# Harrypotterrrr/DVD-GAN

Hardware: AMD Instinct MI355X
Metric: clips/sec per G+Ds+Dt step, 48x64x64 UCF-101 synth (higher is better)
Workload: dtype bf16; 1 GPU; UCF-101-shaped 101-class 48x64x64 clips, G+Ds+Dt hinge step, ch=32, k_sample=8, batch 64/GPU (BASELINE configs[1]); global_batch=64, parallelism=dp1

## Files before the change

### dvd_gan_amd/csrc/conv_wgrad.hip

```cpp
#include "conv_common.h"
#include "prof.h"
#include <cstdlib>
#include <type_traits>

namespace {

struct WgK {
    const char* x; const char* dy; float* dw;
    int M, C, ldx, Cin_real, Cout, Cy, ldy;
    int T, H, W, logH, logW, Hin, Win;
    int kt, kh, kw, up2, relu_in;
    int tiles_co, tiles_ci, rows_per_split;
    long long s_co, s_ci, s_tap;
    size_t x_bytes, dy_bytes;
    int maxshift, xcd_remap;
    float* dbias;
    float* wsb;
    float* ws;
    int fold, cout_f;
};

template <typename G>
__host__ __device__ __forceinline__ size_t ws_tile_off(size_t slice, G gx, int bx, int kw, int t, int tile_elems) { return ((slice * gx + bx) * kw + t) * (size_t)tile_elems; }
template <typename G>
// ... 3 lines not shown

__device__ __forceinline__ void xcd_block_remap(const WgK& p, int& bx, int& bz) {
    bx = blockIdx.x; bz = blockIdx.z;
    if (p.xcd_remap) {
        const int gx = gridDim.x, total = gx * gridDim.z, lin = bx + gx * bz;
        const int xcd = lin & 7, qd = total >> 3, rr = total & 7;
        const int lp = (xcd < rr ? xcd * (qd + 1) : rr * (qd + 1) + (xcd - rr) * qd) + (lin >> 3);
        bz = lp / gx; bx = lp - bz * gx;
    }
}
__device__ __forceinline__ void bf16x8_unpack(const u32x4& r, float (&v)[8]) {
    v[0] = __uint_as_float(r.x << 16); v[1] = __uint_as_float(r.x & 0xffff0000u);
    v[2] = __uint_as_float(r.y << 16); v[3] = __uint_as_float(r.y & 0xffff0000u);
    v[4] = __uint_as_float(r.z << 16); v[5] = __uint_as_float(r.z & 0xffff0000u);
    v[6] = __uint_as_float(r.w << 16); v[7] = __uint_as_float(r.w & 0xffff0000u);
}
#define WG_BIAS_FINISH(CPRA, RPPA, NV, TAB, TO_WS, N, I)                                                                \
    do {                                                                                                                \
        __syncthreads();                                                                                                \
        if (tid < CPRA) {                                                                                               \
            for (int k = 0; k < NV; ++k) {                                                                              \
                float a = 0.f;                                                                                          \
                for (int r = 0; r < RPPA; ++r) a += TAB;                                                                \
                const int co = co0 + tid * NV + k;                                                                      \
                if (TO_WS) p.wsb[ws_bias_off(bz, N, I, BMc) + tid * NV + k] = a;                                        \
                else if (co < p.Cout && a != 0.f) atomicAdd(p.dbias + co, a);      \
            }                                                                                                           \
        }                                                                                                               \
        __syncthreads();                                                                                                \
    } while (0)
#define WG_TILE_TAIL(ACC, ROW0, COL0, KW_, T, TAP)                                                                      \
    do {                                                                                                                \
        _Pragma("unroll") for (int r = 0; r < 16; ++r)                                                                  \
            ep[((r & 3) + 8 * (r >> 2) + 4 * (lane >> 5)) * 32 + (lane & 31)] = ACC[r];                                 \
        __builtin_amdgcn_s_waitcnt(0xc07f);                                                                             \
        __builtin_amdgcn_wave_barrier();                                                                                \
        const int ci = ci0 + COL0 + (lane & 31);                                                                        \
        const int cob = co0 + ROW0 + (lane >> 5);                                                                       \
        const int wtap = TAP;                   \
        if (p.ws) {                                                                                                     \
            float* wt = p.ws + ws_tile_off(bz, gridDim.x, bx, KW_, T, BMc * BNc) + (size_t)(ROW0) * BNc + COL0;         \
            _Pragma("unroll 1") for (int j = 0; j < 16; ++j)                                                            \
                wt[(size_t)(2 * j + (lane >> 5)) * BNc + (lane & 31)] = ep[(2 * j + (lane >> 5)) * 32 + (lane & 31)];   \
        } else if (ci < p.Cin_real) {                                                                                   \
            float* dst = p.dw + ci * p.s_ci + wtap * p.s_tap;                                                           \
            _Pragma("unroll 1") for (int j = 0; j < 16; ++j) {                                                          \
                const int co = cob + 2 * j;                                                                             \
                const float v = ep[(2 * j + (lane >> 5)) * 32 + (lane & 31)];                                           \
                if (co < p.Cout && v != 0.f) atomicAdd(dst + co * p.s_co, v);                                           \
            }                                                                                                           \
        }                                                                                                               \
        __builtin_amdgcn_wave_barrier();                                                                                \
    } while (0)
template <typename T, int TA, int TB>
__global__ __launch_bounds__(NT) void conv_wgrad_kernel(WgK p) {
    constexpr bool kBf16 = sizeof(T) == 2;
    static_assert(kBf16 || (TA == 2 && TB == 2), "exact mode uses the 128 x 128 tile");
    constexpr int BKW = kBf16 ? 32 : 16;
    constexpr int BMc = TA * 64, BNc = TB * 64;
    constexpr int RSA = BMc * 2 + 64, RSB = BNc * 2 + 64;
    constexpr int TA_BYTES = kBf16 ? 32 * RSA : TILEB, TB_BYTES = kBf16 ? 32 * RSB : TILEB;
    __shared__ __attribute__((aligned(16))) char smem[2][TA_BYTES + TB_BYTES];
    const int tid = threadIdx.x, lane = tid & 63, wave = tid >> 6;
    const int wm = wave >> 1, wn = wave & 1;
    int bx, bz;
    xcd_block_remap(p, bx, bz);
    const int tiles = p.tiles_co * p.tiles_ci;
    const int tap = bx / tiles;
    const int rem = bx - tap * tiles;
    const int tco = rem / p.tiles_ci, tci = rem - tco * p.tiles_ci;
    const int co0 = tco * BMc, ci0 = tci * BNc;
    const int it = tap / (p.kh * p.kw), r2 = tap - it * p.kh * p.kw;
    const int iy = r2 / p.kw, ix = r2 - iy * p.kw;
    const int dt = it - (p.kt >> 1), dy_ = iy - (p.kh >> 1), dx = ix - (p.kw >> 1);
    const int m_begin = bz * p.rows_per_split;
    const int m_end = min(p.M, m_begin + p.rows_per_split);

    f32x16 acc[TA][TB];
    {
        const f32x16 zacc = {0.f, 0.f, 0.f, 0.f, 0.f, 0.f, 0.f, 0.f, 0.f, 0.f, 0.f, 0.f, 0.f, 0.f, 0.f, 0.f};
#pragma unroll
        for (int a = 0; a < TA; ++a)
#pragma unroll
            for (int b = 0; b < TB; ++b) acc[a][b] = zacc;
    }

    constexpr unsigned ESZ = sizeof(T);
    const int xbase_row = p.up2 ? (m_begin / (p.H * p.W)) * p.Hin * p.Win : max(0, m_begin - p.maxshift);
    const size_t xbase_b = (size_t)xbase_row * p.ldx * ESZ, ybase_b = (size_t)m_begin * p.ldy * ESZ;
    const size_t xleft = p.x_bytes - xbase_b, yleft = p.dy_bytes > ybase_b ? p.dy_bytes - ybase_b : 0;
    const __amdgpu_buffer_rsrc_t rx = __builtin_amdgcn_make_buffer_rsrc(
        (void*)(p.x + xbase_b), 0, xleft > 0xfffffffeull ? 0xfffffffeu : (unsigned)xleft, 0x00020000);
    const __amdgpu_buffer_rsrc_t rdy = __builtin_amdgcn_make_buffer_rsrc(
        (void*)(p.dy + ybase_b), 0, yleft > 0xfffffffeull ? 0xfffffffeu : (unsigned)yleft, 0x00020000);
    const int delta = (dt * p.H + dy_) * p.W + dx;
    auto xoff = [&](int m, unsigned chan_bytes, bool cvalid) __attribute__((always_inline)) -> unsigned {
        int fm, ym, xm;
        grid_pos(m, p.H, p.W, p.logH, p.logW, fm, ym, xm);
        const int xx = xm + dx, yy = ym + dy_;
        int tt = dt;
        if (p.kt > 1) tt += fm % p.T;
        const bool ok = cvalid && m < m_end && (unsigned)yy < (unsigned)p.H && (unsigned)xx < (unsigned)p.W &&
                        (unsigned)tt < (unsigned)p.T;
        int row = m + delta;
        if (p.up2) row = ((fm + dt) * p.Hin + (yy >> 1)) * p.Win + (xx >> 1);
        return ok ? (unsigned)(row - xbase_row) * ((unsigned)p.ldx * ESZ) + chan_bytes : 0xffffffffu;
// ... 428 lines not shown
#pragma unroll
        for (int s_ = 0; s_ < NS; ++s_) mma1(&smem[buf * STAGE + s_ * SUB]);
    };
    if (m_begin < m_end) {
        const bool late = NWAVE == 8 && NS == 2 && wave >= 4;
        gload(m_begin);
        lstore(0);
        if (late) gload(m_begin + 32 * NS);
        __builtin_amdgcn_s_waitcnt(0xc07f);
        __builtin_amdgcn_s_barrier();
        int buf = 0;
        for (int mk = m_begin; mk < m_end; mk += 32 * NS, buf ^= 1) {
            if (!late) {
                gload(mk + 32 * NS);
                mma(buf);
                lstore(buf ^ 1);
            } else {
                mma1(&smem[buf * STAGE]);
                lstore(buf ^ 1);
                gload(mk + 2 * 32 * NS);
                mma1(&smem[buf * STAGE + (NS - 1) * SUB]);
            }
            __builtin_amdgcn_s_waitcnt(0xc07f);
            __builtin_amdgcn_s_barrier();
        }
        __builtin_amdgcn_s_waitcnt(0x0070);
    }
    if (do_bias) {
        float* red = reinterpret_cast<float*>(&smem[0]);
#pragma unroll
        for (int k = 0; k < 8; ++k) red[tid * 8 + k] = bs[k];
        WG_BIAS_FINISH(CPRA, RPPA, 8, red[(r * CPRA + tid) * 8 + k], spread, gridDim.x, bx);
    }
    float* ep = reinterpret_cast<float*>(&smem[0]) + wave * (32 * 32);
#pragma unroll
    for (int a = 0; a < 2; ++a)
#pragma unroll
        for (int t = 0; t < KW; ++t)
            WG_TILE_TAIL(acc[a][t], wm * 64 + a * 32, wn * 32, KW, t, irow * KW + t);
}
template <int I, int N, typename F>
__device__ __forceinline__ void static_for(F&& f) {
    if constexpr (I < N) {
        f(std::integral_constant<int, I>{});
        static_for<I + 1, N>(f);
    }
}
template <bool V>
__device__ __forceinline__ void mfma_pinned(f32x16& c, const bf16x8& a, const bf16x8& b) {
    if constexpr (V) asm volatile("v_mfma_f32_32x32x16_bf16 %0, %1, %2, %0" : "+v"(c) : "v"(a), "v"(b));
    else asm volatile("v_mfma_f32_32x32x16_bf16 %0, %1, %2, %0" : "+a"(c) : "v"(a), "v"(b));
}

#ifndef DVD_EXP_ROW4
#define DVD_EXP_ROW4 0
#endif
template <int KW, int AW, int BW, int WCO, int WCI, bool RELU, int DEPTH = 2, bool FOLD = false>
__global__ __launch_bounds__(256) void conv_wgrad_row4_kernel(WgK p) {
    constexpr bool BLDS = KW == 3 && AW * BW * KW > 16 && DEPTH >= 2;
    static_assert(WCO * WCI == 4, "four waves, one per SIMD");
    constexpr int NTt = 256, BMc = WCO * AW * 32, NHB = WCI * BW, BNc = NHB * 32;
    constexpr int RSA = BMc * 2 + 64;
    constexpr int TA_BYTES = 32 * RSA;
    constexpr int XROWS = KW == 5 ? 64 : 48, XHALF = XROWS * 64, TB_BYTES = NHB * XHALF;
    constexpr int SUB = TA_BYTES + TB_BYTES;
    constexpr int EPIB = 4 * 32 * 32 * 4, REDB = NTt * 8 * 4;
    constexpr int LDSB0 = 3 * SUB > EPIB ? (3 * SUB > REDB ? 3 * SUB : REDB) : (EPIB > REDB ? EPIB : REDB);
    constexpr int LDSB = LDSB0 + (BLDS ? REDB : 0);
    __shared__ __attribute__((aligned(16))) char smem[LDSB];
    const int tid = threadIdx.x, lane = tid & 63, wave = tid >> 6;
    const int wm = wave / WCI, wn = wave % WCI;
    int bx = blockIdx.x, bz = blockIdx.z;
    if (p.xcd_remap) {
        const int gx = gridDim.x, total = gx * gridDim.z, lin = bx + gx * bz;
        const int xcd = lin & 7, qd = total >> 3, rr = total & 7;
        const int lp = (xcd < rr ? xcd * (qd + 1) : rr * (qd + 1) + (xcd - rr) * qd) + (lin >> 3);
        bz = lp / gx; bx = lp - bz * gx;
    }
    const int tiles = p.tiles_co * p.tiles_ci;
    const int irow = bx / tiles;
    const int rem = bx - irow * tiles;
    const int tco = rem / p.tiles_ci, tci = rem - tco * p.tiles_ci;
    const int co0 = tco * BMc, ci0 = tci * BNc;
    constexpr int pad = KW >> 1;
    static_assert(!FOLD || (KW == 3 && BMc == 128), "the folded form runs on the 3-tap 128-channel tile");
    const int it = FOLD ? 0 : irow / KW, iy = FOLD ? irow : irow - it * KW;
    const int dyl = FOLD ? ((co0 / p.cout_f) >> 1) - 1 + irow : iy - pad, dtl = FOLD ? 0 : it - (p.kt >> 1);
    const int m_begin = bz * p.rows_per_split;
    const int m_end = min(p.M, m_begin + p.rows_per_split);

    f32x16 acc[AW][BW][KW];
    {
        const f32x16 zacc = {0.f, 0.f, 0.f, 0.f, 0.f, 0.f, 0.f, 0.f, 0.f, 0.f, 0.f, 0.f, 0.f, 0.f, 0.f, 0.f};
#pragma unroll
        for (int a = 0; a < AW; ++a)
#pragma unroll
            for (int b = 0; b < BW; ++b)
#pragma unroll
                for (int t = 0; t < KW; ++t) acc[a][b][t] = zacc;
    }
    const int xbase_row = max(0, m_begin - p.maxshift);
    const int ybase_row = FOLD ? 4 * m_begin - 2 * (p.W > 32 ? m_begin & (p.W - 1) : 0) : m_begin;
    const size_t xbase_b = (size_t)xbase_row * p.ldx * 2, ybase_b = (size_t)ybase_row * p.ldy * 2;
    const size_t xleft = p.x_bytes - xbase_b, yleft = p.dy_bytes > ybase_b ? p.dy_bytes - ybase_b : 0;
    const __amdgpu_buffer_rsrc_t rx = __builtin_amdgcn_make_buffer_rsrc(
        (void*)(p.x + xbase_b), 0, xleft > 0xfffffffeull ? 0xfffffffeu : (unsigned)xleft, 0x00020000);
    const __amdgpu_buffer_rsrc_t rdy = __builtin_amdgcn_make_buffer_rsrc(
        (void*)(p.dy + ybase_b), 0, yleft > 0xfffffffeull ? 0xfffffffeu : (unsigned)yleft, 0x00020000);
    const int segw = min(p.W, 32), logsegw = min(p.logW, 5);
    const int fpr = segw + KW - 1, frows = (32 >> logsegw) * fpr;
    constexpr int CPRA = BMc / 8, RPPA = NTt / CPRA, NPA = 32 / RPPA;
    const int rra = tid / CPRA, cka = tid % CPRA;
    const int cy = co0 + cka * 8;
    const bool cyv = cy < p.Cy;
    constexpr int CPX = NHB * 4;
    constexpr int NXL = (XROWS * CPX + NTt - 1) / NTt;
    constexpr int NOPS = NPA + NXL;
    constexpr bool XFULL = NXL * NTt == XROWS * CPX;
    int xa[NXL];
    static_assert(NTt % CPX == 0, "chunk i of a thread sits NTt / CPX footprint rows below chunk i - 1");
    const int xdst0 = ((tid % CPX) >> 2) * XHALF + (tid / CPX) * 64 + ((tid % CPX) & 3) * 16;
    unsigned xld[NXL];
    bool xv[NXL];
    const bool twofr = (32 >> logsegw) > p.H;
    const bool wide = p.W > 32;
    const unsigned ldx2 = (unsigned)p.ldx * 2, ldy2 = (unsigned)p.ldy * 2;
#pragma unroll
    for (int i = 0; i < NXL; ++i) {
        const int q = tid + i * NTt, row = q / CPX, c8 = q % CPX;
        const int seg = row / fpr, j = row - seg * fpr;
        const int cx = ci0 + c8 * 8;
        const int fo = twofr ? seg >> p.logH : 0, yl = twofr ? seg & (p.H - 1) : seg;
        const int xya = yl + dyl, xxa = j - pad;
        xa[i] = wide ? xxa : xya;
        xv[i] = row < frows && cx < p.C && (wide || (unsigned)xxa < (unsigned)p.W);
        const int delta = (fo << (p.logW + p.logH)) + (xya << p.logW) + xxa;
        xld[i] = (unsigned)delta * ldx2 + (unsigned)cx * 2;
    }
    unsigned yld = (unsigned)rra * ldy2 + (unsigned)cy * 2;
    unsigned ystep = (unsigned)RPPA * ldy2;
    if constexpr (FOLD) {
        static_assert(!FOLD || RPPA == 16, "16 rows per staging pass");
        const int ph = cy / p.cout_f, c = cy - ph * p.cout_f, W2 = 2 * p.W;
        yld = (unsigned)(((rra >> logsegw) * 2 + (ph >> 1)) * W2 + 2 * (rra & (segw - 1)) + (ph & 1)) * ldy2 + (unsigned)c * 2;
        ystep = (unsigned)(segw == 32 ? 32 : (16 >> logsegw) * 2 * W2) * ldy2;
    }
    const int dt_rows = p.kt > 1 ? dtl << (p.logW + p.logH) : 0;
    u32x4 R[DEPTH][NOPS];
    struct Geo { int sval; unsigned xoff, yoff; bool tok, ytok; };
    const unsigned slim = wide ? p.W : p.H;
    auto geo_part = [&](Geo& g, int mk, int part) __attribute__((always_inline)) {
        if (part == 0) {
            const int x0 = mk & (p.W - 1), y = twofr ? 0 : (mk >> p.logW) & (p.H - 1);
            g.sval = wide ? x0 : y;
            g.ytok = mk < m_end;
            g.tok = g.ytok && (!wide || (unsigned)(y + dyl) < (unsigned)p.H);
        } else if (part == 1) {
            if (p.kt > 1) {
                const int tt = (mk >> (p.logW + p.logH)) % p.T + dtl;
                g.tok = g.tok && (unsigned)tt < (unsigned)p.T;
            }
        } else if (part == 2) {
            g.xoff = (unsigned)(mk + dt_rows - xbase_row) * ldx2;
        } else {
// ... 43 lines not shown
            for (int k = 0; k < 8; ++k) {
                if constexpr (BLDS) __hip_atomic_fetch_add(btab + k * NTt, v8[k], __ATOMIC_RELAXED, __HIP_MEMORY_SCOPE_WORKGROUP);
                else bs[k] += v8[k];
            }
            return;
        }
        if (op < NPA) {
            *reinterpret_cast<u32x4*>(st + (rra + op * RPPA) * RSA + cka * 16) = R[op];
            if (mine) {
                float v[8];
                bf16x8_unpack(R[op], v);
#pragma unroll
                for (int k = 0; k < 8; ++k) {
                    if constexpr (BLDS) __hip_atomic_fetch_add(btab + k * NTt, v[k], __ATOMIC_RELAXED, __HIP_MEMORY_SCOPE_WORKGROUP);
                    else bs[k] += v[k];
                }
            }
        } else {
            const int i = op - NPA;
            if (XFULL || tid + i * NTt < XROWS * CPX)
                *reinterpret_cast<u32x4*>(st + TA_BYTES + xdst0 + i * (NTt / CPX) * 64) = RELU ? relu16_bf16(R[op]) : R[op];
        }
    };
    typedef __attribute__((ext_vector_type(4))) short s16x4;
    typedef __attribute__((ext_vector_type(8))) short s16x8;
    const int g16 = lane >> 4, i16 = lane & 15;
    const int frow = (g16 >> 1) * 8 + (i16 >> 2), fcol2 = ((g16 & 1) * 16 + (i16 & 3) * 4) * 2;
    auto tr2 = [&](const char* lo_, const char* hi_) __attribute__((always_inline)) -> bf16x8 {
        s16x4 lo = __builtin_amdgcn_ds_read_tr16_b64_v4i16((__attribute__((address_space(3))) s16x4*)lo_);
        s16x4 hi = __builtin_amdgcn_ds_read_tr16_b64_v4i16((__attribute__((address_space(3))) s16x4*)hi_);
        s16x8 f = __builtin_shufflevector(lo, hi, 0, 1, 2, 3, 4, 5, 6, 7);
        return __builtin_bit_cast(bf16x8, f);
    };
    const int fr0 = (frow >> logsegw) * fpr + (frow & (segw - 1));
    const int hlstep = (segw >= 8 ? 4 : fpr) * 64;
    const int kbstep = ((16 >> logsegw) * fpr + (16 & (segw - 1))) * 64;
    const int xoff0 = TA_BYTES + wn * BW * XHALF + fr0 * 64 + fcol2;
    const int aoff = frow * RSA + fcol2 + (wm * AW * 32) * 2;
    constexpr int UPK = KW * BW, NU = 2 * UPK;
    constexpr bool PIN = AW * BW * KW > 16;
    constexpr int UB = NU - 2;
    constexpr int RING = NU % 3 == 0 ? 3 : 5;
    static_assert(NU % RING == 0, "B fragment ring");
    bf16x8 fa[AW], fb[RING];
    auto ldA = [&](const char* st, int kb, int a) __attribute__((always_inline)) {
        const char* pz = st + aoff + kb * 16 * RSA + a * 64;
        fa[a] = tr2(pz, pz + 4 * RSA);
    };
    auto ldB = [&](const char* st, int u, int slot) __attribute__((always_inline)) {
        const int kb = u / UPK, t = (u % UPK) / BW, b = u % BW;
        const char* pz = st + xoff0 + kb * kbstep + t * 64 + b * XHALF;
        fb[slot] = tr2(pz, pz + hlstep);
    };
    if (m_begin < m_end) {
        {
            const Geo g0 = geo(m_begin);
#pragma unroll
            for (int op = 0; op < NOPS; ++op) load_op(op, g0, R[0]);
            const bool mine = do_bias && bphase == myshare;
            if (++bphase == nshare) bphase = 0;
#pragma unroll
            for (int op = 0; op < NOPS; ++op) store_op(op, &smem[0], mine, R[0]);
#pragma unroll
            for (int d = 0; d < DEPTH; ++d) {
                const Geo g1 = geo(m_begin + 32 * (d + 1));
#pragma unroll
                for (int op = 0; op < NOPS; ++op) load_op(op, g1, R[d]);
            }
            __builtin_amdgcn_s_waitcnt(0xc07f);
            __builtin_amdgcn_s_barrier();
#pragma unroll
            for (int a = 0; a < AW - 1; ++a) ldA(&smem[0], 0, a);
            ldB(&smem[0], 0, 0);
            ldB(&smem[0], 1, 1);
        }
        char* rd = &smem[0];
        char* nx = &smem[SUB];
        char* fr_ = &smem[2 * SUB];
        static_assert(AW == 4, "slot plan written for four A fragments per wave");
        Geo gl = geo(m_begin + 32 * (DEPTH + 1));
        for (int mk0 = m_begin; mk0 < m_end; mk0 += 32 * DEPTH) {
          static_for<0, DEPTH>([&](auto D_) __attribute__((always_inline)) {
            constexpr int dset = decltype(D_)::value;
            const int mk = mk0 + 32 * dset;
            const bool mine = do_bias && bphase == myshare;
            if (++bphase == nshare) bphase = 0;
            Geo gn = gl;
            __builtin_amdgcn_sched_barrier(0);
            static_for<0, NU * AW>([&](auto S_) __attribute__((always_inline)) {
                constexpr int s = decltype(S_)::value, u = s / AW, a = s % AW;
                constexpr int kb = u / UPK, t = (u % UPK) / BW, b = u % BW;
                if constexpr (u == UB && a == 0) {
                    __builtin_amdgcn_s_waitcnt(0xc07f);
                    if (!(DVD_EXP_ROW4 & 4)) __builtin_amdgcn_s_barrier();
                }
                if constexpr (a == 0) {
                    if (u + 2 < NU) ldB(rd, u + 2, (u + 2) % RING);
                    else ldB(nx, u + 2 - NU, (u + 2) % RING);
                }
                if constexpr (a == 1 || (ST64 && a == 2)) {
#pragma unroll
                    for (int op = 0; op < NOPS; ++op)
                        if ((op * UB) / NOPS == u && !(DVD_EXP_ROW4 & 2)) {
                            if constexpr (ST64) store_op(op, nx, mine, R[dset], a - 1);
                            else store_op(op, nx, mine, R[dset]);
                        }
                }
                if constexpr (u == UPK - 1 && a >= 1) ldA(rd, 1, a - 1);
                if constexpr (u == UPK && a == 0) ldA(rd, 1, AW - 1);
                if constexpr (u == NU - 1 && a >= 1) ldA(nx, 0, a - 1);
                if constexpr (u == 0 && a == 0) ldA(rd, 0, AW - 1);
                if constexpr (a == AW - 1) {
#pragma unroll
                    for (int op = 0; op < NOPS; ++op)
                        if ((op * UB) / NOPS == u && !(DVD_EXP_ROW4 & 1)) load_op(op, gl, R[dset]);
                }
                if constexpr (u == UB - 1 && a == AW - 1) geo_part(gn, mk + 32 * (DEPTH + 2), 0);
                if constexpr (u == UB && a >= 1) geo_part(gn, mk + 32 * (DEPTH + 2), a);
                if constexpr (PIN) mfma_pinned<((a * BW + b) * KW + t >= 16)>(acc[a][b][t], fa[a], fb[u % RING]);
                else acc[a][b][t] = __builtin_amdgcn_mfma_f32_32x32x16_bf16(fa[a], fb[u % RING], acc[a][b][t], 0, 0, 0);
                __builtin_amdgcn_sched_barrier(0);
            });
            gl = gn;
            char* t_ = rd; rd = nx; nx = fr_; fr_ = t_;
          });
        }
        __builtin_amdgcn_s_waitcnt(0x0070);
        if constexpr (PIN) asm volatile("s_nop 15\n\ts_nop 15" ::: "memory");
        __syncthreads();
    }
    if (do_bias) {
        if constexpr (!BLDS) {
#pragma unroll
            for (int k = 0; k < 8; ++k) btab[k * NTt] = bs[k];
        }
        WG_BIAS_FINISH(CPRA, RPPA, 8, btab[k * NTt + r * CPRA], spread, gridDim.x, bx);
    }
    float* ep = reinterpret_cast<float*>(&smem[0]) + wave * (32 * 32);
#pragma unroll
    for (int a = 0; a < AW; ++a)
#pragma unroll
        for (int b = 0; b < BW; ++b)
#pragma unroll
            for (int t = 0; t < KW; ++t)
                WG_TILE_TAIL(acc[a][b][t], (wm * AW + a) * 32, (wn * BW + b) * 32, KW, t, irow * KW + t);
}
#undef WG_BIAS_FINISH
#undef WG_TILE_TAIL
__device__ __forceinline__ f32x4 slice_sum4(const float* ws, int nslice, size_t stride, size_t off) {
    f32x4 a = {0.f, 0.f, 0.f, 0.f};
    int z = 0;
    for (; z + 4 <= nslice; z += 4) {
        f32x4 v[4];
#pragma unroll
        for (int j = 0; j < 4; ++j) v[j] = *reinterpret_cast<const f32x4*>(ws + (size_t)(z + j) * stride + off);
#pragma unroll
        for (int j = 0; j < 4; ++j) a += v[j];
    }
    for (; z < nslice; ++z) a += *reinterpret_cast<const f32x4*>(ws + (size_t)z * stride + off);
    return a;
}
__device__ __forceinline__ void wg_store4(float* d, long long s_ci, int ci, int Cin_real, const f32x4& a, int overwrite) {
#pragma unroll
    for (int j = 0; j < 4; ++j)
        if (ci + j < Cin_real) d[j * s_ci] = overwrite ? a[j] : d[j * s_ci] + a[j];
}
template <typename F>
__device__ __forceinline__ float block_sum_32x32(int nitem, F&& item) {
    __shared__ float red[32][33];
    const int c = threadIdx.x & 31, l = threadIdx.x >> 5;
    float a = 0.f;
    for (int i = l; i < nitem; i += 32 * 8) {
        float v[8];
#pragma unroll
        for (int u = 0; u < 8; ++u) v[u] = i + 32 * u < nitem ? item(i + 32 * u) : 0.f;
#pragma unroll
        for (int u = 0; u < 8; ++u) a += v[u];
    }
    red[l][c] = a;
    __syncthreads();
    if (l == 0)
        for (int j = 1; j < 32; ++j) a += red[j][c];
    return a;
}

struct WgRowRedK { const float* ws; float* dw; int nslice, gx, tiles_co, tiles_ci, BMc, BNc, KW, Cout, Cin_real; long long s_co, s_ci, s_tap; int overwrite; };
__global__ void wgrad_row_reduce_kernel(WgRowRedK p) {
    const int tile = p.BMc * p.BNc, tile_elems = p.KW * tile;
    const long long i = ((long long)blockIdx.x * blockDim.x + threadIdx.x) * 4;
    if (i >= (long long)p.gx * tile_elems) return;
    const int bx = (int)(i / tile_elems), e = (int)(i - (long long)bx * tile_elems);
    const int t = e / tile, e2 = e - t * tile;
    const int r = e2 / p.BNc, c = e2 - r * p.BNc;
    const int tiles = p.tiles_co * p.tiles_ci;
    const int iy = bx / tiles, rem = bx - iy * tiles;
    const int tco = rem / p.tiles_ci, tci = rem - tco * p.tiles_ci;
    const int co = tco * p.BMc + r, ci = tci * p.BNc + c;
    if (co >= p.Cout || ci >= p.Cin_real) return;
    const f32x4 a = slice_sum4(p.ws, p.nslice, ws_slice_stride(p.gx, p.KW, tile), ws_tile_off(0, p.gx, bx, p.KW, t, tile) + e2);
    wg_store4(p.dw + co * p.s_co + ci * p.s_ci + (iy * p.KW + t) * p.s_tap, p.s_ci, ci, p.Cin_real, a, p.overwrite);
}
// ... 39 lines not shown
    const int ci4 = (p.Cin_real + 3) / 4;
    const long long i = (long long)blockIdx.x * blockDim.x + threadIdx.x;
    if (i >= (long long)9 * p.Cout * ci4) return;
    const int cq = (int)(i % ci4), rest = (int)(i / ci4);
    const int co = rest % p.Cout, tap = rest / p.Cout;
    const int ky = tap / 3 - 1, kx = tap % 3 - 1, ci = cq * 4;
    const int tiles = (4 * p.Cout / 128) * p.tiles_ci;
    f32x4 acc = {0.f, 0.f, 0.f, 0.f};
#pragma unroll
    for (int ph = 0; ph < 4; ++ph) {
        const int a = ph >> 1, b = ph & 1;
        const int sy = (a + ky) >> 1, sx = (b + kx) >> 1;
        const int irow = sy - a + 1, t = sx + 1;
        const int cop = ph * p.Cout + co;
        const int bx = irow * tiles + (cop >> 7) * p.tiles_ci + (ci >> 7);
        const size_t off = ws_tile_off(0, p.gx, bx, 3, t, 128 * 128) + (size_t)(cop & 127) * 128 + (ci & 127);
        acc += slice_sum4(p.ws, p.nslice, ws_slice_stride(p.gx, 3, 128 * 128), off);
    }
    wg_store4(p.dw + co * p.s_co + ci * p.s_ci + tap * p.s_tap, p.s_ci, ci, p.Cin_real, acc, p.overwrite);
}
struct WgFoldBiasK { const float* wsb; float* dbias; int nslice, gx, tiles_ci, Cout; };
__global__ __launch_bounds__(1024) void wgrad_fold_bias_reduce_kernel(WgFoldBiasK p) {
    const int co = blockIdx.x * 32 + (threadIdx.x & 31);
    const int tiles = (4 * p.Cout / 128) * p.tiles_ci, per = 2 * p.tiles_ci;
    const float a = block_sum_32x32(4 * p.nslice * per, [&](int i) __attribute__((always_inline)) -> float {
        if (co >= p.Cout) return 0.f;
        const int ph = i / (p.nslice * per), r0 = i - ph * (p.nslice * per);
        const int bz = r0 / per, r = r0 - bz * per;
        const int irow = r / p.tiles_ci, tci = r - irow * p.tiles_ci;
        const int cop = ph * p.Cout + co;
        const int bx = irow * tiles + (cop >> 7) * p.tiles_ci + tci;
        return p.wsb[ws_bias_off(bz, p.gx, bx, 128) + (cop & 127)];
    });
    if (threadIdx.x < 32 && co < p.Cout) p.dbias[co] += a;
}

constexpr long long WG_TGT_TAP = 2048, WG_MINROWS = 4096;
constexpr long long WG_TGT_ROW = 512;
constexpr long long WG_TGT_ROW64 = 768;
constexpr long long WG_TGT_ROW4 = 256, WG_TGT_ROW4_LARGE = 512, WG_ROW4_LARGE_M = 6ll << 20;
constexpr long long WG_ROW4_MIN_WGS = 224, WG_ROW4_WG_ROWS = 4096;
constexpr long long WG_CUS = 256;

enum WgFamily { WG_TAP = 0, WG_ROW = 1, WG_ROW4 = 2 };

struct WgPlan {
    int rc;
    WgK p;
    dim3 grid;
    WgFamily family;
    int bm, bn;
    int kw_tile, esz;
    int depth, fold;
    long long msplit;
    long long tile_floats, bias_floats;
    long long total() const { return tile_floats + bias_floats; }
    long long base() const { return (long long)p.tiles_co * p.tiles_ci * (family == WG_TAP ? p.kt * p.kh * p.kw : fold ? 2 : p.kt * p.kh); }
};

}

static int wg_fill_request(const dvd_wgrad_desc* d, WgPlan& pl) {
    if (!d || !d->x || !d->dy || !d->dw) return DVD_E_ARG;
    int logH = ilog2_exact(d->H), logW = ilog2_exact(d->W);
    if (logH < 0 || logW < 0) logH = logW = -1;
    if (d->up2 && ((d->H | d->W) & 1)) return DVD_E_SHAPE;
    if ((d->C & 7) || (d->ldx & 7) || (d->Cy & 7) || (d->ldy & 7) || !(d->kt & d->kh & d->kw & 1)) return DVD_E_SHAPE;
    if (d->Cout > d->Cy || d->Cin_real > d->C) return DVD_E_ARG;
    if (d->dtype != DVD_BF16 && d->dtype != DVD_F32) return DVD_E_ARG;
    const long long M = (long long)d->frames * d->T * d->H * d->W;
    if (M >= (1ll << 31) - 64) return DVD_E_SHAPE;
    WgK& p = pl.p;
    p.x = (const char*)d->x; p.dy = (const char*)d->dy; p.dw = d->dw;
    p.M = (int)M; p.C = d->C; p.ldx = d->ldx; p.Cin_real = d->Cin_real; p.Cout = d->Cout; p.Cy = d->Cy; p.ldy = d->ldy;
    p.T = d->T; p.H = d->H; p.W = d->W; p.logH = logH; p.logW = logW;
    p.Hin = d->up2 ? d->H / 2 : d->H; p.Win = d->up2 ? d->W / 2 : d->W;
    p.kt = d->kt; p.kh = d->kh; p.kw = d->kw; p.up2 = d->up2; p.relu_in = d->relu_in;
    p.s_co = d->s_co; p.s_ci = d->s_ci; p.s_tap = d->s_tap; p.dbias = d->dbias; p.ws = nullptr; p.wsb = nullptr;
    p.xcd_remap = 1;
    p.fold = 0; p.cout_f = d->Cout;
    pl.esz = d->dtype == DVD_BF16 ? 2 : 4;
    const size_t rows_in = (size_t)d->frames * d->T * p.Hin * p.Win;
    p.x_bytes = ((rows_in - 1) * (size_t)d->ldx + d->C) * pl.esz;
    p.dy_bytes = (((size_t)M - 1) * (size_t)d->ldy + d->Cy) * pl.esz;
    p.maxshift = ((d->kt >> 1) * d->H + (d->kh >> 1)) * d->W + (d->kw >> 1);
    return DVD_OK;
}

static int wg_choose_tile(const dvd_wgrad_desc* d, bool fold, WgPlan& pl) {
    const WgK& p = pl.p;
    const bool bf16 = d->dtype == DVD_BF16, pow2 = p.logW >= 0;
    pl.family = WG_TAP; pl.bm = 128; pl.bn = 128; pl.depth = 0; pl.fold = fold;
    if (bf16) {
        if (d->Cout >= 192) pl.bm = 256;
        else if (d->Cin_real >= 192) pl.bn = 256;
    }
    const bool row = pow2 && bf16 && d->kh == d->kw && (d->kw == 3 || d->kw == 5) && (!d->up2 || (d->kw == 3 && d->kt == 1)) &&
                     ((d->W >= 8 && (d->H * d->W) % 32 == 0) ||
                      (d->W == 4 && d->H == 4 && d->kt == 1 && d->T == 1 && !d->up2 && (d->frames & 1) == 0));
    if (row) {
        const int w4 = (d->Cout + 255) / 256 * 256, w2 = (d->Cout + 127) / 128 * 128;
        pl.family = WG_ROW;
        pl.bm = d->Cout <= 64 ? 64 : (w4 <= w2 ? 256 : 128); pl.bn = 64;
        const bool ci128 = (d->Cin_real + 127) / 128 * 128 == (d->Cin_real + 63) / 64 * 64;
        if (pl.bm == 128 && d->kw == 5 && !d->up2 && ci128) pl.bn = 128;
        if (!d->up2 && pl.bm >= 128 && (d->kw == 3 ? ci128 : (pl.bm == 256 || ci128))) {
            int bm4 = pl.bm, bn4 = 128;
            if (d->kw == 3) { if (fold) bm4 = 128; }
            else if (pl.bm == 256) bn4 = 64;
            const long long wgs = (long long)((d->Cout + bm4 - 1) / bm4) * ((d->Cin_real + bn4 - 1) / bn4) * d->kt * d->kh * (p.M / WG_ROW4_WG_ROWS);
            if (wgs >= WG_ROW4_MIN_WGS || d->msplit > 0) {
                pl.family = WG_ROW4; pl.bm = bm4; pl.bn = bn4;
                pl.depth = (d->kw == 3 && bm4 == 256 && d->dbias) ? 1 : 2;
            }
        }
    }
    if (fold && pl.family != WG_ROW4) return DVD_E_SHAPE;
    pl.p.tiles_co = (d->Cout + pl.bm - 1) / pl.bm; pl.p.tiles_ci = (d->Cin_real + pl.bn - 1) / pl.bn;
    return DVD_OK;
}

static long long wg_split_target(const WgPlan& pl) {
    const long long tgt = pl.family == WG_ROW4 ? (pl.p.M > WG_ROW4_LARGE_M ? WG_TGT_ROW4_LARGE : WG_TGT_ROW4)
                        : pl.family == WG_ROW  ? (pl.bm == 64 ? WG_TGT_ROW64 : WG_TGT_ROW)
                                               : WG_TGT_TAP;
    return (tgt + pl.base() - 1) / pl.base();
}
static long long wg_split_cap(const WgPlan& pl) {
    const long long M = pl.p.M, base = pl.base();
    long long cap = M / WG_MINROWS > 0 ? M / WG_MINROWS : 1;
    if (pl.p.kt * pl.p.kh * pl.p.kw == 1 && cap * base < 256) {
        const long long want = (256 + base - 1) / base, cap2 = M / 256;
        cap = cap2 < want ? (cap2 > cap ? cap2 : cap) : want;
    }
    return cap;
}
static void wg_choose_split(const dvd_wgrad_desc* d, WgPlan& pl) {
    const bool automatic = d->msplit < 1;
    const long long M = pl.p.M, base = pl.base();
    long long msplit = d->msplit;
    if (automatic) {
        const long long cap = wg_split_cap(pl);
        msplit = wg_split_target(pl);
        if (msplit > cap) msplit = cap;
        const int per_cu = (pl.family != WG_TAP && (pl.bm == 256 || pl.bn == 128)) ? 1 : (pl.family == WG_ROW && pl.bm == 64) ? 3 : 2;
        const long long conc = WG_CUS * per_cu;
        if (base * msplit > conc) {
            const long long rounds = (base * msplit + conc / 2) / conc;
            const long long ms2 = rounds * conc / base;
            if (ms2 >= 1 && ms2 <= cap) msplit = ms2;
        }
    }
    long long rows = (M + msplit - 1) / msplit;
    const long long ldy_eff = pl.fold ? 4ll * d->ldy : d->ldy;
    const long long rowcap = (1ll << 31) / ((d->ldx > ldy_eff ? d->ldx : ldy_eff) * pl.esz);
    if (rows > rowcap) rows = rowcap;
    rows = (rows + 31) / 32 * 32;
    if (rows < 32) rows = 32;
    msplit = (M + rows - 1) / rows;
    const long long wg = base * msplit;
    if (automatic && pl.family == WG_ROW4 && wg > WG_CUS && wg % WG_CUS > 0 && wg % WG_CUS < 192) {
        const long long ms2 = ((wg + WG_CUS - 1) / WG_CUS * WG_CUS) / base;
        if (ms2 > msplit && M / ms2 >= 2048) {
            rows = ((M + ms2 - 1) / ms2 + 31) / 32 * 32;
            msplit = (M + rows - 1) / rows;
        }
    }
    pl.msplit = msplit;
    pl.p.rows_per_split = (int)rows;
    pl.grid = dim3((unsigned)base, 1, (unsigned)msplit);
}

static WgPlan wgrad_plan(const dvd_wgrad_desc* d, bool may_fold) {
    WgPlan pl{};
    auto plan1 = [&pl](const dvd_wgrad_desc* q, bool fold) {
        int rc = wg_fill_request(q, pl);
        if (rc == DVD_OK) rc = wg_choose_tile(q, fold, pl);
        if (rc == DVD_OK) wg_choose_split(q, pl);
        return rc;
    };
    pl.rc = DVD_E_SHAPE;
    if (may_fold && d && d->up2 && d->dtype == DVD_BF16 && d->kt == 1 && d->kh == 3 && d->kw == 3 && d->T == 1 &&
        d->Cout % 64 == 0 && d->Cy >= d->Cout && !((d->H | d->W) & 1)) {
        dvd_wgrad_desc e = *d;
        e.H = d->H / 2; e.W = d->W / 2; e.up2 = 0;
        e.Cout = e.Cy = 4 * d->Cout;
        pl.rc = plan1(&e, true);
        if (pl.rc == DVD_OK) {
            const size_t M4 = (size_t)d->frames * d->T * d->H * d->W;
            pl.p.dy_bytes = ((M4 - 1) * (size_t)d->ldy + d->Cy) * 2;
            pl.p.fold = 1; pl.p.cout_f = d->Cout;
        }
    }
    if (pl.rc != DVD_OK) pl.rc = plan1(d, false);
    if (pl.rc != DVD_OK) return pl;
    pl.kw_tile = pl.family == WG_TAP ? 1 : d->kw;
    pl.tile_floats = (long long)ws_tile_off(pl.msplit, pl.grid.x, 0, pl.kw_tile, 0, pl.bm * pl.bn);
    pl.bias_floats = (long long)ws_bias_off(pl.msplit, pl.family == WG_TAP ? (unsigned)pl.p.tiles_co : pl.grid.x, 0, pl.bm);
    return pl;
}

extern "C" long long dvd_conv_wgrad_ws_floats(const dvd_wgrad_desc* d) {
    if (const long long thin = dvd_wgrad_thin_ws_floats(d)) return thin;
    const WgPlan pl = wgrad_plan(d, true);
    if (pl.rc != DVD_OK || (pl.msplit <= 1 && !pl.fold)) return 0;
    return pl.total();
}

namespace {

template <int WM, int KW, bool UP2 = false, int NH = 2>
void launch_row(const WgPlan& pl, hipStream_t st) {
    if (pl.p.relu_in) conv_wgrad_row_kernel<WM, KW, true, UP2, NH><<<pl.grid, WM * NH * 64, 0, st>>>(pl.p);
    else conv_wgrad_row_kernel<WM, KW, false, UP2, NH><<<pl.grid, WM * NH * 64, 0, st>>>(pl.p);
}
template <int KW, int AW, int BW, int WCO, int WCI, int DEPTH, bool FOLD = false>
void launch_row4(const WgPlan& pl, hipStream_t st) {
    if (pl.p.relu_in) conv_wgrad_row4_kernel<KW, AW, BW, WCO, WCI, true, DEPTH, FOLD><<<pl.grid, 256, 0, st>>>(pl.p);
    else conv_wgrad_row4_kernel<KW, AW, BW, WCO, WCI, false, DEPTH, FOLD><<<pl.grid, 256, 0, st>>>(pl.p);
}

constexpr unsigned wg_key(WgFamily family, int bm, int bn, int kw, int up2, int depth, int fold, int f32 = 0) {
    return (unsigned)family | (bm / 64) << 2 | (bn / 64) << 5 | kw << 8 | up2 << 11 | depth << 12 | fold << 14 | f32 << 15;
}

bool wg_launch(const WgPlan& pl, hipStream_t st) {
    const bool tap = pl.family == WG_TAP;
    switch (wg_key(pl.family, pl.bm, pl.bn, tap ? 0 : pl.p.kw, tap ? 0 : pl.p.up2 != 0, pl.depth, pl.fold, tap && pl.esz == 4)) {
    case wg_key(WG_TAP,  256, 128, 0, 0, 0, 0):    conv_wgrad_kernel<bf16_t, 4, 2><<<pl.grid, NT, 0, st>>>(pl.p); break;
    case wg_key(WG_TAP,  128, 256, 0, 0, 0, 0):    conv_wgrad_kernel<bf16_t, 2, 4><<<pl.grid, NT, 0, st>>>(pl.p); break;
    case wg_key(WG_TAP,  128, 128, 0, 0, 0, 0):    conv_wgrad_kernel<bf16_t, 2, 2><<<pl.grid, NT, 0, st>>>(pl.p); break;
    case wg_key(WG_TAP,  128, 128, 0, 0, 0, 0, 1): conv_wgrad_kernel<float, 2, 2><<<pl.grid, NT, 0, st>>>(pl.p); break;
    case wg_key(WG_ROW,   64,  64, 3, 0, 0, 0):    launch_row<1, 3>(pl, st); break;
    case wg_key(WG_ROW,   64,  64, 5, 0, 0, 0):    launch_row<1, 5>(pl, st); break;
    case wg_key(WG_ROW,  128,  64, 3, 0, 0, 0):    launch_row<2, 3>(pl, st); break;
    case wg_key(WG_ROW,  128,  64, 5, 0, 0, 0):    launch_row<2, 5>(pl, st); break;
    case wg_key(WG_ROW,  256,  64, 3, 0, 0, 0):    launch_row<4, 3>(pl, st); break;
    case wg_key(WG_ROW,  256,  64, 5, 0, 0, 0):    launch_row<4, 5>(pl, st); break;
    case wg_key(WG_ROW,   64,  64, 3, 1, 0, 0):    launch_row<1, 3, true>(pl, st); break;
    case wg_key(WG_ROW,  128,  64, 3, 1, 0, 0):    launch_row<2, 3, true>(pl, st); break;
    case wg_key(WG_ROW,  256,  64, 3, 1, 0, 0):    launch_row<4, 3, true>(pl, st); break;
    case wg_key(WG_ROW,  128, 128, 3, 0, 0, 0):    launch_row<2, 3, false, 4>(pl, st); break;
    case wg_key(WG_ROW,  128, 128, 5, 0, 0, 0):    launch_row<2, 5, false, 4>(pl, st); break;
    case wg_key(WG_ROW4, 256, 128, 3, 0, 1, 0):    launch_row4<3, 4, 2, 2, 2, 1>(pl, st); break;
    case wg_key(WG_ROW4, 256, 128, 3, 0, 2, 0):    launch_row4<3, 4, 2, 2, 2, 2>(pl, st); break;
    case wg_key(WG_ROW4, 128, 128, 3, 0, 2, 0):    launch_row4<3, 4, 1, 1, 4, 2>(pl, st); break;
    case wg_key(WG_ROW4, 128, 128, 3, 0, 2, 1):    launch_row4<3, 4, 1, 1, 4, 2, true>(pl, st); break;
    case wg_key(WG_ROW4, 256,  64, 5, 0, 2, 0):    launch_row4<5, 4, 1, 2, 2, 2>(pl, st); break;
    case wg_key(WG_ROW4, 128, 128, 5, 0, 2, 0):    launch_row4<5, 4, 1, 1, 4, 2>(pl, st); break;
    default: return false;
    }
    return true;
}

}

extern "C" int dvd_conv_wgrad(const dvd_wgrad_desc* d, void* stream) {
    WgPlan pl = wgrad_plan(d, d && d->ws != nullptr);
    if (pl.rc != DVD_OK) return pl.rc;
    WgK& p = pl.p;
    hipStream_t st = (hipStream_t)stream;
    const int ntaps = d->kt * d->kh * d->kw, nslice = (int)pl.msplit, gx = (int)pl.grid.x;
    const long long Mreal = (long long)d->frames * d->T * d->H * d->W;
    if (d->ws && dvd_wgrad_thin_ws_floats(d)) {
        if (d->overwrite && (d->s_tap != 1 || d->s_ci != ntaps || d->s_co != (long long)d->Cin_real * ntaps)) return DVD_E_ARG;
        ProfScope prof(1, 2.0 * (double)Mreal * d->Cout * d->Cin_real * ntaps, stream, (int)Mreal, d->C, d->Cout, ntaps, 0, d->relu_in << 1);
        prof.r.variant = 3;
        return dvd_wgrad_thin(d, stream);
    }
    if (d->ws && (pl.msplit > 1 || pl.fold)) {
        p.ws = d->ws;
        p.wsb = d->ws + pl.tile_floats;
    }
    const int overwrite = d->overwrite != 0;
    if (overwrite) {
        if (d->s_tap != 1 || d->s_ci != ntaps || d->s_co != (long long)d->Cin_real * ntaps) return DVD_E_ARG;
        if (!p.ws && hipMemsetAsync(d->dw, 0, (size_t)d->Cout * d->Cin_real * ntaps * sizeof(float), st) != hipSuccess)
            return DVD_E_LAUNCH;
    }
    ProfScope prof(1, 2.0 * (double)Mreal * d->Cout * d->Cin_real * ntaps, stream, (int)Mreal, d->C, d->Cout, ntaps, nslice,
                   d->up2 | (d->relu_in << 1));
    prof.r.variant = pl.family == WG_ROW4 ? 4 : pl.family == WG_ROW ? 1 : 2;
    if (!wg_launch(pl, st)) return DVD_E_SHAPE;
    if (!p.ws) return launch_status();
    if (pl.fold) {
        WgFoldRedK r{p.ws, p.dw, nslice, gx, p.tiles_ci, d->Cout, p.Cin_real, p.s_co, p.s_ci, p.s_tap, overwrite};
        wgrad_fold_reduce_kernel<<<cdiv(9ll * d->Cout * ((p.Cin_real + 3) / 4), 256), 256, 0, st>>>(r);
        if (p.dbias) {
            WgFoldBiasK b{p.wsb, p.dbias, nslice, gx, p.tiles_ci, d->Cout};
            wgrad_fold_bias_reduce_kernel<<<cdiv(d->Cout, 32), 1024, 0, st>>>(b);
        }
        return launch_status();
    }
    WgRowRedK r{p.ws, p.dw, nslice, gx, p.tiles_co, p.tiles_ci, pl.bm, pl.bn, pl.kw_tile, p.Cout, p.Cin_real, p.s_co, p.s_ci, p.s_tap, overwrite};
    const long long n = pl.tile_floats / nslice;
    wgrad_row_reduce_kernel<<<cdiv(n / 4, 256), 256, 0, st>>>(r);
    if (p.dbias) {
        if (pl.family == WG_TAP) wgrad_bias_reduce_kernel<<<cdiv(p.Cout, 64), 1024, 0, st>>>(p.wsb, p.dbias, nslice, p.tiles_co, pl.bm, p.Cout);
        else {
            WgBiasRedK b{p.wsb, p.dbias, nslice, gx, p.tiles_co, p.tiles_ci, d->kw, d->kt, pl.bm, p.Cout};
            wgrad_row_bias_reduce_kernel<<<p.tiles_co * (pl.bm / 32), 1024, 0, st>>>(b);
// ... 5 lines not shown
```

Measured before the change: 147.1 clips/s.

## Add direct-register A operand path for 5-tap 256x64 row4 wgrad kernel

Adds a DIRECT variant of the row4 weight-gradient kernel for kw=5, 256x64 tiles. It loads dy straight from global memory into registers and builds the MFMA A fragments with byte permutes, so the LDS staging for the A tile is gone. It uses four waves along Cout with a three-deep pipeline, a rowmapped epilogue and a separate bias reduction. This removes LDS traffic and A-side barriers, at the cost of more VGPR pressure and uncoalesced 32-bit global loads. It is on by default and can be disabled with DVD_WG_DIRECT=0.

```diff
diff --git a/dvd_gan_amd/csrc/conv_wgrad.hip b/dvd_gan_amd/csrc/conv_wgrad.hip
--- a/dvd_gan_amd/csrc/conv_wgrad.hip
+++ b/dvd_gan_amd/csrc/conv_wgrad.hip
@@ -79,6 +79,29 @@
         }                                                                                                               \
         __builtin_amdgcn_wave_barrier();                                                                                \
     } while (0)
+#define WG_TILE_TAIL_ROWMAP(ACC, WROW0, A_, COL0, KW_, T, TAP)                                                          \
+    do {                                                                                                                \
+        _Pragma("unroll") for (int r = 0; r < 16; ++r)                                                                  \
+            ep[((r & 3) + 8 * (r >> 2) + 4 * (lane >> 5)) * 32 + (lane & 31)] = ACC[r];                                 \
+        __builtin_amdgcn_s_waitcnt(0xc07f);                                                                             \
+        __builtin_amdgcn_wave_barrier();                                                                                \
+        const int ci = ci0 + COL0 + (lane & 31);                                                                        \
+        const int rowb = WROW0 + A_ + 2 * (lane >> 5);         \
+        const int wtap = TAP;                                                                                           \
+        if (p.ws) {                                                                                                     \
+            float* wt = p.ws + ws_tile_off(bz, gridDim.x, bx, KW_, T, BMc * BNc) + COL0;                                \
+            _Pragma("unroll 1") for (int j = 0; j < 16; ++j)                                                            \
+                wt[(size_t)(rowb + 4 * j) * BNc + (lane & 31)] = ep[(2 * j + (lane >> 5)) * 32 + (lane & 31)];          \
+        } else if (ci < p.Cin_real) {                                                                                   \
+            float* dst = p.dw + ci * p.s_ci + wtap * p.s_tap;                                                           \
+            _Pragma("unroll 1") for (int j = 0; j < 16; ++j) {                                                          \
+                const int co = co0 + rowb + 4 * j;                                                                      \
+                const float v = ep[(2 * j + (lane >> 5)) * 32 + (lane & 31)];                                           \
+                if (co < p.Cout && v != 0.f) atomicAdd(dst + co * p.s_co, v);                                           \
+            }                                                                                                           \
+        }                                                                                                               \
+        __builtin_amdgcn_wave_barrier();                                                                                \
+    } while (0)
 template <typename T, int TA, int TB>
 __global__ __launch_bounds__(NT) void conv_wgrad_kernel(WgK p) {
     constexpr bool kBf16 = sizeof(T) == 2;
@@ -613,16 +636,23 @@
     else asm volatile("v_mfma_f32_32x32x16_bf16 %0, %1, %2, %0" : "+a"(c) : "v"(a), "v"(b));
 }
 
+#ifndef DVD_DIRECT_AHEAD
+#define DVD_DIRECT_AHEAD 2
+#endif
+#ifndef DVD_DIRECT_DEPTH
+#define DVD_DIRECT_DEPTH 3
+#endif
 #ifndef DVD_EXP_ROW4
 #define DVD_EXP_ROW4 0
 #endif
-template <int KW, int AW, int BW, int WCO, int WCI, bool RELU, int DEPTH = 2, bool FOLD = false>
+template <int KW, int AW, int BW, int WCO, int WCI, bool RELU, int DEPTH = 2, bool FOLD = false, bool DIRECT = false>
 __global__ __launch_bounds__(256) void conv_wgrad_row4_kernel(WgK p) {
+    static_assert(!DIRECT || (KW == 5 && AW == 2 && BW == 2 && WCO == 4 && WCI == 1 && (DEPTH == 2 || DEPTH == 3) && !FOLD), "the direct-A form: 5 taps, 256 x 64");
     constexpr bool BLDS = KW == 3 && AW * BW * KW > 16 && DEPTH >= 2;
     static_assert(WCO * WCI == 4, "four waves, one per SIMD");
     constexpr int NTt = 256, BMc = WCO * AW * 32, NHB = WCI * BW, BNc = NHB * 32;
     constexpr int RSA = BMc * 2 + 64;
-    constexpr int TA_BYTES = 32 * RSA;
+    constexpr int TA_BYTES = DIRECT ? 0 : 32 * RSA;
     constexpr int XROWS = KW == 5 ? 64 : 48, XHALF = XROWS * 64, TB_BYTES = NHB * XHALF;
     constexpr int SUB = TA_BYTES + TB_BYTES;
     constexpr int EPIB = 4 * 32 * 32 * 4, REDB = NTt * 8 * 4;
@@ -670,7 +700,7 @@
         (void*)(p.dy + ybase_b), 0, yleft > 0xfffffffeull ? 0xfffffffeu : (unsigned)yleft, 0x00020000);
     const int segw = min(p.W, 32), logsegw = min(p.logW, 5);
     const int fpr = segw + KW - 1, frows = (32 >> logsegw) * fpr;
-    constexpr int CPRA = BMc / 8, RPPA = NTt / CPRA, NPA = 32 / RPPA;
+    constexpr int CPRA = BMc / 8, RPPA = NTt / CPRA, NPA = DIRECT ? 0 : 32 / RPPA;
     const int rra = tid / CPRA, cka = tid % CPRA;
     const int cy = co0 + cka * 8;
     const bool cyv = cy < p.Cy;
@@ -820,7 +850,114 @@
         const char* pz = st + xoff0 + kb * kbstep + t * 64 + b * XHALF;
         fb[slot] = tr2(pz, pz + hlstep);
     };
-    if (m_begin < m_end) {
+    if constexpr (DIRECT) {
+        static_assert(!DIRECT || (NXL == 2 && XFULL && UPK == 10 && RING == 5 && PIN && ST64), "slot plan of the direct-A form");
+        unsigned Y[DEPTH][16];
+        const int cyd = co0 + wm * 64 + 2 * (lane & 31);
+        const bool cydv = cyd < p.Cy;
+        const unsigned yldd = (unsigned)((lane >> 5) * 8) * ldy2 + (unsigned)cyd * 2;
+        auto loadY = [&](int q, unsigned yv, unsigned (&Ys)[16]) __attribute__((always_inline)) {
+            if (!(DVD_EXP_ROW4 & 1)) Ys[q] = __builtin_amdgcn_raw_buffer_load_b32(rdy, yv, (unsigned)((q >> 3) * 16 + (q & 7)) * ldy2, 0);
+        };
+        constexpr int AH = DVD_DIRECT_AHEAD;
+        static_assert(RING >= AH + 2, "the ring holds the units read ahead, the current one and the one still kept");
+        bf16x8 fd[2][2];
+        auto mkA = [&](int kb, int a, const unsigned (&Ys)[16]) __attribute__((always_inline)) {
+            u32x4 v;
+#pragma unroll
+            for (int m = 0; m < 4; ++m)
+                v[m] = __builtin_amdgcn_perm(Ys[kb * 8 + 2 * m + 1], Ys[kb * 8 + 2 * m], a ? 0x07060302u : 0x05040100u);
+            asm volatile("" : "+v"(v));
+            fd[kb][a] = __builtin_bit_cast(bf16x8, v);
+        };
+        auto keep = [&](const bf16x8& v) __attribute__((always_inline)) { asm volatile("" ::"v"(v)); };
+        auto biasY = [&](int kb, const unsigned (&Ys)[16]) __attribute__((always_inline)) {
+#pragma unroll
+            for (int e = 0; e < 8; ++e) {
+                bs[0] += __uint_as_float(Ys[kb * 8 + e] << 16);
+                bs[1] += __uint_as_float(Ys[kb * 8 + e] & 0xffff0000u);
+            }
+        };
+        if (m_begin < m_end) {
+            {
+                const Geo g0 = geo(m_begin);
+#pragma unroll
+                for (int op = 0; op < NOPS; ++op) load_op(op, g0, R[0]);
+#pragma unroll
+                for (int q = 0; q < 16; ++q) Y[0][q] = __builtin_amdgcn_raw_buffer_load_b32(rdy, cydv && g0.ytok ? yldd + (unsigned)((q >> 3) * 16 + (q & 7)) * ldy2 : 0xffffffffu, 0, 0);
+#pragma unroll
+                for (int op = 0; op < NOPS; ++op) store_op(op, &smem[0], false, R[0]);
+#pragma unroll
+                for (int d = 0; d < DEPTH; ++d) {
+                    const Geo g1 = geo(m_begin + 32 * (d + 1));
+#pragma unroll
+                    for (int op = 0; op < NOPS; ++op) load_op(op, g1, R[d]);
+                }
+#pragma unroll
+                for (int d = 1; d < DEPTH; ++d)
+#pragma unroll
+                    for (int q = 0; q < 16; ++q)
+                        Y[d][q] = __builtin_amdgcn_raw_buffer_load_b32(rdy, cydv && m_begin + 32 * d < m_end ? yldd + (unsigned)(32 * d + (q >> 3) * 16 + (q & 7)) * ldy2 : 0xffffffffu, 0, 0);
+                __builtin_amdgcn_s_waitcnt(0xc07f);
+                __builtin_amdgcn_s_barrier();
+                mkA(0, 0, Y[0]);
+                mkA(0, 1, Y[0]);
+                const bf16x8 zf = __builtin_bit_cast(bf16x8, u32x4{0u, 0u, 0u, 0u});
+                fd[1][0] = fd[1][1] = zf;
+#pragma unroll
+                for (int i = AH; i < RING; ++i) fb[i] = zf;
+#pragma unroll
+                for (int i = 0; i < AH; ++i) ldB(&smem[0], i, i);
+            }
+            char* rd = &smem[0];
+            char* nx = &smem[SUB];
+            char* fr_ = &smem[2 * SUB];
+            Geo gl = geo(m_begin + 32 * (DEPTH + 1));
+            for (int mk0 = m_begin; mk0 < m_end; mk0 += 32 * DEPTH) {
+              static_for<0, DEPTH>([&](auto D_) __attribute__((always_inline)) {
+                constexpr int dset = decltype(D_)::value;
+                const int mk = mk0 + 32 * dset;
+                const bool mine = do_bias && bphase == myshare;
+                if (++bphase == nshare) bphase = 0;
+                const unsigned yv2 = cydv && mk + 32 * DEPTH < m_end ? yldd + (unsigned)(mk + 32 * DEPTH - m_begin) * ldy2 : 0xffffffffu;
+                Geo gn = gl;
+                __builtin_amdgcn_sched_barrier(0);
+                static_for<0, NU * AW>([&](auto S_) __attribute__((always_inline)) {
+                    constexpr int s = decltype(S_)::value, u = s / AW, a = s % AW;
+                    constexpr int kb = u / UPK, t = (u % UPK) / BW, b = u % BW;
+                    constexpr int s2 = (s + NU * AW - 2) % (NU * AW), u2 = s2 / AW;
+                    keep(fd[u2 / UPK][s2 % AW]);
+                    keep(fb[u2 % RING]);
+                    if constexpr (a == 0) {
+                        if constexpr (u == NU - AH) {
+                            __builtin_amdgcn_s_waitcnt(0xc07f);
+                            if (!(DVD_EXP_ROW4 & 4)) __builtin_amdgcn_s_barrier();
+                        }
+                        if (u + AH < NU) ldB(rd, u + AH, (u + AH) % RING);
+                        else ldB(nx, u + AH - NU, (u + AH) % RING);
+                        if constexpr (u >= 2 && u < 6 && !(DVD_EXP_ROW4 & 2)) store_op((u - 2) >> 1, nx, false, R[dset], (u - 2) & 1);
+                        if constexpr ((u == 6 || u == 7) && !(DVD_EXP_ROW4 & 1)) load_op(u - 6, gl, R[dset]);
+                        if constexpr (u >= 12 && u < 16) geo_part(gn, mk + 32 * (DEPTH + 2), u - 12);
+                        if constexpr (u == 0 || u == UPK - 1) {
+                            if (mine) biasY(u == 0 ? 0 : 1, Y[dset]);
+                        }
+                    } else {
+                        if constexpr (u % UPK < 8) loadY(kb * 8 + u % UPK, yv2, Y[dset]);
+                        if constexpr (u == UPK - 2 || u == UPK - 1) mkA(1, u - (UPK - 2), Y[dset]);
+                        if constexpr (u == NU - 2 || u == NU - 1) mkA(0, u - (NU - 2), Y[(dset + 1) % DEPTH]);
+                    }
+                    mfma_pinned<((a * BW + b) * KW + t >= 16)>(acc[a][b][t], fd[kb][a], fb[u % RING]);
+                    __builtin_amdgcn_sched_barrier(0);
+                });
+                gl = gn;
+                char* t_ = rd; rd = nx; nx = fr_; fr_ = t_;
+              });
+            }
+            __builtin_amdgcn_s_waitcnt(0x0070);
+            asm volatile("s_nop 15\n\ts_nop 15" ::: "memory");
+            __syncthreads();
+        }
+    } else if (m_begin < m_end) {
         {
             const Geo g0 = geo(m_begin);
 #pragma unroll
@@ -897,7 +1034,21 @@
         if constexpr (PIN) asm volatile("s_nop 15\n\ts_nop 15" ::: "memory");
         __syncthreads();
     }
-    if (do_bias) {
+    if constexpr (DIRECT) {
+        if (do_bias) {
+            float* tab = reinterpret_cast<float*>(&smem[0]);
+            const int c2 = wm * 64 + 2 * (lane & 31);
+            tab[(lane >> 5) * BMc + c2] = bs[0];
+            tab[(lane >> 5) * BMc + c2 + 1] = bs[1];
+            __syncthreads();
+            static_assert(!DIRECT || BMc == NTt, "one thread per channel of the tile");
+            const float a = tab[tid] + tab[BMc + tid];
+            const int co = co0 + tid;
+            if (spread) p.wsb[ws_bias_off(bz, gridDim.x, bx, BMc) + tid] = a;
+            else if (co < p.Cout && a != 0.f) atomicAdd(p.dbias + co, a);
+            __syncthreads();
+        }
+    } else if (do_bias) {
         if constexpr (!BLDS) {
 #pragma unroll
             for (int k = 0; k < 8; ++k) btab[k * NTt] = bs[k];
@@ -910,11 +1061,14 @@
 #pragma unroll
         for (int b = 0; b < BW; ++b)
 #pragma unroll
-            for (int t = 0; t < KW; ++t)
-                WG_TILE_TAIL(acc[a][b][t], (wm * AW + a) * 32, (wn * BW + b) * 32, KW, t, irow * KW + t);
+            for (int t = 0; t < KW; ++t) {
+                if constexpr (DIRECT) WG_TILE_TAIL_ROWMAP(acc[a][b][t], wm * 64, a, (wn * BW + b) * 32, KW, t, irow * KW + t);
+                else WG_TILE_TAIL(acc[a][b][t], (wm * AW + a) * 32, (wn * BW + b) * 32, KW, t, irow * KW + t);
+            }
 }
 #undef WG_BIAS_FINISH
 #undef WG_TILE_TAIL
+#undef WG_TILE_TAIL_ROWMAP
 __device__ __forceinline__ f32x4 slice_sum4(const float* ws, int nslice, size_t stride, size_t off) {
     f32x4 a = {0.f, 0.f, 0.f, 0.f};
     int z = 0;
@@ -1060,6 +1214,7 @@
     int bm, bn;
     int kw_tile, esz;
     int depth, fold;
+    int direct;
     long long msplit;
     long long tile_floats, bias_floats;
     long long total() const { return tile_floats + bias_floats; }
@@ -1095,10 +1250,15 @@
     return DVD_OK;
 }
 
+static bool wg_direct_enabled() {
+    const char* e = std::getenv("DVD_WG_DIRECT");
+    return !(e && e[0] == '0' && e[1] == 0);
+}
+
 static int wg_choose_tile(const dvd_wgrad_desc* d, bool fold, WgPlan& pl) {
     const WgK& p = pl.p;
     const bool bf16 = d->dtype == DVD_BF16, pow2 = p.logW >= 0;
-    pl.family = WG_TAP; pl.bm = 128; pl.bn = 128; pl.depth = 0; pl.fold = fold;
+    pl.family = WG_TAP; pl.bm = 128; pl.bn = 128; pl.depth = 0; pl.fold = fold; pl.direct = 0;
     if (bf16) {
         if (d->Cout >= 192) pl.bm = 256;
         else if (d->Cin_real >= 192) pl.bn = 256;
@@ -1120,6 +1280,7 @@
             if (wgs >= WG_ROW4_MIN_WGS || d->msplit > 0) {
                 pl.family = WG_ROW4; pl.bm = bm4; pl.bn = bn4;
                 pl.depth = (d->kw == 3 && bm4 == 256 && d->dbias) ? 1 : 2;
+                pl.direct = d->kw == 5 && bm4 == 256 && bn4 == 64 && wg_direct_enabled();
             }
         }
     }
@@ -1222,19 +1383,19 @@
     if (pl.p.relu_in) conv_wgrad_row_kernel<WM, KW, true, UP2, NH><<<pl.grid, WM * NH * 64, 0, st>>>(pl.p);
     else conv_wgrad_row_kernel<WM, KW, false, UP2, NH><<<pl.grid, WM * NH * 64, 0, st>>>(pl.p);
 }
-template <int KW, int AW, int BW, int WCO, int WCI, int DEPTH, bool FOLD = false>
+template <int KW, int AW, int BW, int WCO, int WCI, int DEPTH, bool FOLD = false, bool DIRECT = false>
 void launch_row4(const WgPlan& pl, hipStream_t st) {
-    if (pl.p.relu_in) conv_wgrad_row4_kernel<KW, AW, BW, WCO, WCI, true, DEPTH, FOLD><<<pl.grid, 256, 0, st>>>(pl.p);
-    else conv_wgrad_row4_kernel<KW, AW, BW, WCO, WCI, false, DEPTH, FOLD><<<pl.grid, 256, 0, st>>>(pl.p);
-}
-
-constexpr unsigned wg_key(WgFamily family, int bm, int bn, int kw, int up2, int depth, int fold, int f32 = 0) {
-    return (unsigned)family | (bm / 64) << 2 | (bn / 64) << 5 | kw << 8 | up2 << 11 | depth << 12 | fold << 14 | f32 << 15;
+    if (pl.p.relu_in) conv_wgrad_row4_kernel<KW, AW, BW, WCO, WCI, true, DEPTH, FOLD, DIRECT><<<pl.grid, 256, 0, st>>>(pl.p);
+    else conv_wgrad_row4_kernel<KW, AW, BW, WCO, WCI, false, DEPTH, FOLD, DIRECT><<<pl.grid, 256, 0, st>>>(pl.p);
+}
+
+constexpr unsigned wg_key(WgFamily family, int bm, int bn, int kw, int up2, int depth, int fold, int f32 = 0, int direct = 0) {
+    return (unsigned)family | (bm / 64) << 2 | (bn / 64) << 5 | kw << 8 | up2 << 11 | depth << 12 | fold << 14 | f32 << 15 | direct << 16;
 }
 
 bool wg_launch(const WgPlan& pl, hipStream_t st) {
     const bool tap = pl.family == WG_TAP;
-    switch (wg_key(pl.family, pl.bm, pl.bn, tap ? 0 : pl.p.kw, tap ? 0 : pl.p.up2 != 0, pl.depth, pl.fold, tap && pl.esz == 4)) {
+    switch (wg_key(pl.family, pl.bm, pl.bn, tap ? 0 : pl.p.kw, tap ? 0 : pl.p.up2 != 0, pl.depth, pl.fold, tap && pl.esz == 4, pl.direct)) {
     case wg_key(WG_TAP,  256, 128, 0, 0, 0, 0):    conv_wgrad_kernel<bf16_t, 4, 2><<<pl.grid, NT, 0, st>>>(pl.p); break;
     case wg_key(WG_TAP,  128, 256, 0, 0, 0, 0):    conv_wgrad_kernel<bf16_t, 2, 4><<<pl.grid, NT, 0, st>>>(pl.p); break;
     case wg_key(WG_TAP,  128, 128, 0, 0, 0, 0):    conv_wgrad_kernel<bf16_t, 2, 2><<<pl.grid, NT, 0, st>>>(pl.p); break;
@@ -1255,6 +1416,7 @@
     case wg_key(WG_ROW4, 128, 128, 3, 0, 2, 0):    launch_row4<3, 4, 1, 1, 4, 2>(pl, st); break;
     case wg_key(WG_ROW4, 128, 128, 3, 0, 2, 1):    launch_row4<3, 4, 1, 1, 4, 2, true>(pl, st); break;
     case wg_key(WG_ROW4, 256,  64, 5, 0, 2, 0):    launch_row4<5, 4, 1, 2, 2, 2>(pl, st); break;
+    case wg_key(WG_ROW4, 256,  64, 5, 0, 2, 0, 0, 1): launch_row4<5, 2, 2, 4, 1, DVD_DIRECT_DEPTH, false, true>(pl, st); break;
     case wg_key(WG_ROW4, 128, 128, 5, 0, 2, 0):    launch_row4<5, 4, 1, 1, 4, 2>(pl, st); break;
     default: return false;
     }
```

Result: no change. 147.7 clips/s, median of 6 (+0.5%).
